# delldu/MaskRCNN

Hardware: AMD Instinct MI355X
Metric: images/sec at 1024x1024, 1000 proposals/img (Mask R-CNN inference hot path) (higher is better)
Workload: dtype f32

## Files before the change

__graft_entry__.py:

```python
import importlib.util
import os
import sys

ROOT = os.path.dirname(os.path.abspath(__file__))
if ROOT not in sys.path:
    sys.path.insert(0, ROOT)


def _load(path, name):
    spec = importlib.util.spec_from_file_location(name, path)
    mod = importlib.util.module_from_spec(spec)
    spec.loader.exec_module(mod)
    return mod


def build() -> None:
    import threading
    from oracle import build_ref, oracle

    def _oracles():
        oracle.build()
        try:
            build_ref.build()
        except Exception as e:
            print(f"[build] oracle/_ref not built: {e}", file=sys.stderr)

    t = threading.Thread(target=_oracles)
    t.start()
    b = _load(os.path.join(ROOT, "maskrcnn_amd", "build.py"), "_mrcnn_build")
    b.build_many([(None, (), ()), ("sync_fuzz", ("-DMRCNN_SYNC_FUZZ", "-DMRCNN_W4_ABLATIONS"), ())])
    _load(os.path.join(ROOT, "maskrcnn", "build_native.py"), "_mrcnn_build_native").build()
    t.join()
    import maskrcnn
    import maskrcnn_amd


def smoke() -> None:
    import torch
    assert torch.cuda.is_available(), "smoke() needs a GPU"
    import maskrcnn
    from maskrcnn_amd import modules, ops
    from maskrcnn_amd.config import InferenceConfig
    from maskrcnn_amd.pipeline import MaskRCNNInference
    from oracle import oracle
    dev = torch.device("cuda:0")
    g = torch.Generator().manual_seed(0)
    c = torch.rand(500, 2, generator=g) * 200
    d = torch.cat([c, c + torch.rand(500, 2, generator=g) * 60 + 2,
                   (torch.randperm(500, generator=g).float() / 500)[:, None]], 1)
    assert torch.equal(maskrcnn.nms(d.to(dev), 0.7).cpu(), oracle.nms(d, 0.7)), "nms mismatch"
    img = torch.randn(1, 32, 24, 24, generator=g)
    bx = torch.rand(16, 4, generator=g)
    bx = torch.cat([torch.minimum(bx[:, :2], bx[:, 2:]), torch.maximum(bx[:, :2], bx[:, 2:])], 1)
    ind = torch.zeros(16, dtype=torch.int32)
    got = maskrcnn.CropFunction(7, 7, 0)(img.to(dev), bx.to(dev), ind.to(dev)).cpu()
    assert torch.equal(got, oracle.crop_forward(img, bx, ind, 0.0, 7, 7)), "crop mismatch"
    cfg = InferenceConfig(image_height=128, image_width=128, backbone="resnet50", pre_nms_limit=100,
                          proposal_count=50, detection_max_instances=10)
    sd = modules.synthetic_state_dict("resnet50")
    net = MaskRCNNInference(sd, cfg, dev)
    x = torch.randn(1, 3, 128, 128, generator=g)
    det, mid = net.predict(x.to(dev), torch.tensor([[0., 0., 128., 128.]], device=dev),
                           return_intermediates=True)
    torch.cuda.synchronize()
    want = oracle.fpn_forward(x, sd, "resnet50")
    worst, rng = 0.0, 0.0
    for w, gt in zip(want, mid["feature_maps"]):
        err = (gt[0].permute(2, 0, 1).cpu() - w[0]).abs().max().item()
        worst, rng = max(worst, err), max(rng, w.abs().max().item())
        assert err <= 1e-4, f"trunk mismatch: max|err| {err:.3e} > 1e-4 abs (max|act| {w.abs().max().item():.2f})"
    print(f"trunk vs oracle: max|err| {worst:.2e} abs at max|act| {rng:.2f}")
    assert det.class_ids.shape == (1, 10) and det.masks.shape == (1, 10, 28, 28, 81)
    print("smoke ok")


if __name__ == "__main__":
    build()
    if "--smoke" in sys.argv:
        smoke()
```

maskrcnn_amd/csrc/conv.hip:

```cpp
#include "conv_common.hpp"

#include <algorithm>
#include <cstdlib>
#include <type_traits>

namespace {

using namespace mrcnn_conv;

struct ConvParams : ConvCommon {
    const float* w;
    const float* w_head;
    int head_n;
};

template <int BM, int BN, int BK>
constexpr size_t conv_lds_bytes() {
    return sizeof(float) * 2 * (BM + BN) * (BK == 16 ? BK : BK + 4);
}

template <int BM, int BN, int WM, int WN, int BK, int MODE, int RES, bool SPLIT = false>
__global__ __launch_bounds__(256, 2) void conv_igemm_f32(const ConvParams p) {
    constexpr bool GENERIC = MODE == 1, PW = MODE == 2;
    constexpr bool SWZ = BK == 16;
    constexpr int LDS_STRIDE = SWZ ? BK : BK + 4;
    constexpr int WTM = BM / WM, WTN = BN / WN;
    constexpr int TM = WTM / 32, TN = WTN / 32;
    constexpr int TPR = BK / 4;
    constexpr int RPP = 256 / TPR;
    constexpr int PA = BM / RPP, PB = BN / RPP;
    static_assert(WM * WN == 4 && TM >= 1 && TN >= 1 && PA >= 1 && PB >= 1, "4 waves");
    extern __shared__ __attribute__((aligned(16))) float smem[];
    float* As = smem;
    float* Bs = smem + 2 * BM * LDS_STRIDE;

    int m0, n0, nt;
    if (!tile_origin(p, BM, BN, m0, n0, nt)) return;
    if (p.row_counts && !tile_has_rows(p, m0, BM)) return;

    const int tid = threadIdx.x, lane = tid & 63, wave = tid >> 6;
    const int wm = wave / WN, wn = wave % WN;
    const int kq = tid % TPR, r0 = tid / TPR;
    constexpr bool EARLY_AFFINE = RES == 0 || RES == 3 || RES == 4;
    AffineRegs<TN> affine;
    if constexpr (EARLY_AFFINE) load_affine<TN, WTN>(p, n0, wn, lane, affine);

    int a_off[PA], a_iy[PA], a_ix[PA];
    row_setup<PA, RPP>(p, m0, r0, a_off, a_iy, a_ix);
    int b_off[PB];
    bool b_ok[PB];
#pragma unroll
    for (int i = 0; i < PB; ++i) {
        const int n = n0 + r0 + RPP * i;
        b_ok[i] = n < p.Cout;
        b_off[i] = (b_ok[i] ? n : 0) * p.K + kq * 4;
    }

    unsigned a_voff[PW ? PA : 1], b_voff[PW ? PB : 1];
    if constexpr (PW) {
#pragma unroll
        for (int i = 0; i < PA; ++i)
            a_voff[i] = (m0 + r0 + RPP * i) < p.M ? static_cast<unsigned>(a_off[i] + kq * 4) * 4u : OOB;
#pragma unroll
        for (int i = 0; i < PB; ++i) b_voff[i] = b_ok[i] ? static_cast<unsigned>(b_off[i]) * 4u : OOB;
    }
    float4 ra[PA], rb[PB];
    const __amdgpu_buffer_rsrc_t x_rsrc = __builtin_amdgcn_make_buffer_rsrc(
        const_cast<float*>(p.x), 0, p.x_bytes, 0x00020000);
    const __amdgpu_buffer_rsrc_t w_rsrc = __builtin_amdgcn_make_buffer_rsrc(
        const_cast<float*>(p.w), 0, p.w_bytes, 0x00020000);
    auto bload = [](const __amdgpu_buffer_rsrc_t& r, unsigned byte_off) -> float4 {
        const u32x4 v = __builtin_amdgcn_raw_buffer_load_b128(r, static_cast<int>(byte_off), 0, 0);
        return make_float4(__uint_as_float(v.x), __uint_as_float(v.y), __uint_as_float(v.z),
                           __uint_as_float(v.w));
    };
    int t_c0 = 0, t_ky = 0, t_kx = 0, t_k0 = 0;
    int cur_tap_off = 0, cur_ky = 0, cur_kx = 0, cur_k0 = 0;
    bool cur_kvalid = true;
    int n_c = 0, n_ky = 0, n_kx = 0;
    int g_ky = 0, g_kx = 0, g_tap_off = 0;
    bool g_kin = true;
    if constexpr (GENERIC) {
        const int tap = (kq * 4) / p.Cin;
        n_c = kq * 4 - tap * p.Cin;
        n_ky = tap / p.KW;
        n_kx = tap - n_ky * p.KW;
    }
    auto begin_load = [&]() {
        cur_k0 = t_k0;
        cur_kvalid = t_k0 < p.K;
        if constexpr (GENERIC) {
            g_ky = n_ky;
            g_kx = n_kx;
            g_tap_off = (n_ky * p.W + n_kx) * p.Cin + n_c;
            g_kin = (t_k0 + kq * 4) < p.K;
            n_c += BK;
            while (n_c >= p.Cin) {
                n_c -= p.Cin;
                if (++n_kx == p.KW) { n_kx = 0; ++n_ky; }
            }
        }
        if constexpr (!GENERIC) {
            cur_ky = t_ky;
            cur_kx = t_kx;
            cur_tap_off = (t_ky * p.W + t_kx) * p.Cin + t_c0 + kq * 4;
            t_c0 += BK;
            if (t_c0 >= p.Cin) {
                t_c0 = 0;
                if (++t_kx == p.KW) { t_kx = 0; ++t_ky; }
            }
        }
        t_k0 += BK;
    };
    auto load_piece = [&](int pc) {
        if constexpr (PW) {
            const int kk = cur_k0 < p.K ? cur_k0 : p.K - BK;
            const bool isa = pc < PA;
            const u32x4 v = __builtin_amdgcn_raw_buffer_load_b128(isa ? x_rsrc : w_rsrc,
                                                                  static_cast<int>(isa ? a_voff[isa ? pc : 0] : b_voff[isa ? 0 : pc - PA]),
                                                                  kk * 4, 0);
            const float4 f = make_float4(__uint_as_float(v.x), __uint_as_float(v.y), __uint_as_float(v.z),
                                         __uint_as_float(v.w));
            if (isa) ra[isa ? pc : 0] = f;
            else rb[isa ? 0 : pc - PA] = f;
            return;
        }
        if (pc < PA) {
            const int i = pc;
            if constexpr (!GENERIC) {
                const bool ok = cur_kvalid &&
                                static_cast<unsigned>(a_iy[i] + cur_ky) < static_cast<unsigned>(p.H) &&
                                static_cast<unsigned>(a_ix[i] + cur_kx) < static_cast<unsigned>(p.W);
                ra[i] = bload(x_rsrc, ok ? static_cast<unsigned>(a_off[i] + cur_tap_off) * 4u : OOB);
            } else {
                const bool ok = g_kin &&
                                static_cast<unsigned>(a_iy[i] + g_ky) < static_cast<unsigned>(p.H) &&
                                static_cast<unsigned>(a_ix[i] + g_kx) < static_cast<unsigned>(p.W);
                ra[i] = bload(x_rsrc, ok ? static_cast<unsigned>(a_off[i] + g_tap_off) * 4u : OOB);
            }
        } else {
            const int i = pc - PA;
            bool ok = b_ok[i] && cur_kvalid;
            if constexpr (GENERIC) ok = ok && (cur_k0 + kq * 4 < p.K);
            rb[i] = bload(w_rsrc, ok ? static_cast<unsigned>(b_off[i] + cur_k0) * 4u : OOB);
        }
    };
    static_assert(!SWZ || RPP % 16 == 0, "swizzle term must not depend on the piece");
    const int kqs = SWZ ? (kq ^ ((r0 >> 2) & 3)) : kq;
    auto store_piece = [&](int pc, int buf) {
        if (pc < PA)
            *reinterpret_cast<float4*>(As + buf * BM * LDS_STRIDE + (r0 + RPP * pc) * LDS_STRIDE + kqs * 4) = ra[pc];
        else
            *reinterpret_cast<float4*>(Bs + buf * BN * LDS_STRIDE + (r0 + RPP * (pc - PA)) * LDS_STRIDE + kqs * 4) =
                rb[pc - PA];
    };
    constexpr int NP = PA + PB;

    f32x16 acc[TM][TN];
#pragma unroll
    for (int i = 0; i < TM; ++i)
#pragma unroll
        for (int j = 0; j < TN; ++j)
#pragma unroll
            for (int r = 0; r < 16; ++r) acc[i][j][r] = 0.f;

    const int nk = (p.K + BK - 1) / BK;
    constexpr int NCH = BK / 8;
    constexpr int NM = 4 * TM * TN;
    static_assert(NCH >= 2, "needs at least two chunks per k tile");
    begin_load();
#pragma unroll
    for (int pc = 0; pc < NP; ++pc) load_piece(pc);
#pragma unroll
    for (int pc = 0; pc < NP; ++pc) store_piece(pc, 0);
    __syncthreads();
    begin_load();
#pragma unroll
    for (int pc = 0; pc < NP; ++pc) load_piece(pc);

    const int fsw = SWZ ? (((lane & 31) >> 2) & 3) : 0;
    const int frow = (lane & 31) * LDS_STRIDE;
    const int fch0 = (((lane >> 5)) ^ fsw) * 4, fch1 = ((2 + (lane >> 5)) ^ fsw) * 4;
    const int frag = frow + (lane >> 5) * 4;
    const float* Aw = As + wm * WTM * LDS_STRIDE + (SWZ ? frow : frag);
    const float* Bw = Bs + wn * WTN * LDS_STRIDE + (SWZ ? frow : frag);
    float4 fa[2][TM], fb[2][TN];
    auto read_frags = [&](int slot, int buf, int j) {
        const int jo = SWZ ? (j == 0 ? fch0 : fch1) : j * 8;
#pragma unroll
        for (int i = 0; i < TM; ++i)
            fa[slot][i] = *reinterpret_cast<const float4*>(Aw + buf * BM * LDS_STRIDE + i * 32 * LDS_STRIDE + jo);
#pragma unroll
        for (int i = 0; i < TN; ++i)
            fb[slot][i] = *reinterpret_cast<const float4*>(Bw + buf * BN * LDS_STRIDE + i * 32 * LDS_STRIDE + jo);
    };
    read_frags(0, 0, 0);
    f32x16 acc2[SPLIT ? TM : 1][SPLIT ? TN : 1];
    if constexpr (SPLIT) {
#pragma unroll
        for (int i = 0; i < TM; ++i)
#pragma unroll
            for (int j = 0; j < TN; ++j)
#pragma unroll
                for (int r = 0; r < 16; ++r) acc2[i][j][r] = 0.f;
    }
    auto ktile = [&](auto chain_tag, int kt) {
        constexpr int CH = decltype(chain_tag)::value;
        const int buf = kt & 1;
#pragma unroll
        for (int j = 0; j < NCH; ++j) {
            const int cur = j & 1;
            if (j + 1 < NCH) {
                read_frags(cur ^ 1, buf, j + 1);
            } else {
                __syncthreads();
                read_frags(cur ^ 1, buf ^ 1, 0);
                begin_load();
            }
            __builtin_amdgcn_sched_barrier(0);
#pragma unroll
            for (int s = 0; s < 4; ++s) {
#pragma unroll
                for (int i = 0; i < TM; ++i) {
                    const float4 a = fa[cur][i];
                    const float av = s == 0 ? a.x : s == 1 ? a.y : s == 2 ? a.z : a.w;
#pragma unroll
                    for (int jn = 0; jn < TN; ++jn) {
                        const float4 b = fb[cur][jn];
                        const float bv = s == 0 ? b.x : s == 1 ? b.y : s == 2 ? b.z : b.w;
                        if constexpr (SPLIT && CH == 1)
                            acc2[i][jn] = __builtin_amdgcn_mfma_f32_32x32x2f32(av, bv, acc2[i][jn], 0, 0, 0);
                        else
                            acc[i][jn] = __builtin_amdgcn_mfma_f32_32x32x2f32(av, bv, acc[i][jn], 0, 0, 0);
                        const int m = (s * TM + i) * TN + jn;
#pragma unroll
                        for (int pc = m * NP / NM; pc < (m + 1) * NP / NM; ++pc) {
                            if (j == NCH - 2) store_piece(pc, buf ^ 1);
                            if (j == NCH - 1) load_piece(pc);
                        }
                        __builtin_amdgcn_sched_barrier(0);
                    }
                }
            }
        }
    };
    if constexpr (!SPLIT) {
        for (int kt = 0; kt < nk; ++kt) ktile(std::integral_constant<int, 0>{}, kt);
    } else {
        constexpr int TPB = 32 / BK;
        static_assert(BK == 32 || BK == 16, "SPLIT: chains are 32-wide k blocks");
        for (int kt = 0; kt < nk; kt += 2 * TPB) {
#pragma unroll
            for (int u = 0; u < TPB; ++u)
                if (kt + u < nk) ktile(std::integral_constant<int, 0>{}, kt + u);
#pragma unroll
            for (int u = 0; u < TPB; ++u)
                if (kt + TPB + u < nk) ktile(std::integral_constant<int, 1>{}, kt + TPB + u);
        }
#pragma unroll
        for (int i = 0; i < TM; ++i)
#pragma unroll
            for (int j = 0; j < TN; ++j)
#pragma unroll
                for (int r = 0; r < 16; ++r) acc[i][j][r] += acc2[i][j][r];
    }

    if constexpr (RES == 5) {
        static_assert(BM == 128 && BN == 128 && WM == 2 && WN == 2, "heads epilogue is written for the 128x128 tile");
        constexpr int TS = BN + 4;
        const int ln = lane & 31, lh = lane >> 5;
        __syncthreads();
        float* T = smem;
#pragma unroll
        for (int jn = 0; jn < TN; ++jn) {
            const int n = n0 + wn * WTN + jn * 32 + ln;
            const float sc = p.scale ? p.scale[n] : 1.0f, sh = p.shift ? p.shift[n] : 0.0f;
#pragma unroll
            for (int i = 0; i < TM; ++i)
#pragma unroll
                for (int r = 0; r < 16; ++r) {
                    float v = acc[i][jn][r] * sc + sh;
                    v = v > 0.f ? v : 0.f;
                    T[(wm * WTM + i * 32 + (r & 3) + 8 * (r >> 2) + 4 * lh) * TS + wn * WTN + jn * 32 + ln] = v;
                }
        }
        __syncthreads();
        f32x16 hacc;
#pragma unroll
        for (int r = 0; r < 16; ++r) hacc[r] = 0.f;
        const float* Trow = T + (wave * 32 + ln) * TS + lh * 4;
        const float* Wrow = p.w_head + static_cast<int64_t>(ln) * p.Cout + n0 + lh * 4;
#pragma unroll 4
        for (int j = 0; j < BN / 8; ++j) {
            const float4 a = *reinterpret_cast<const float4*>(Trow + j * 8);
            const float4 b = *reinterpret_cast<const float4*>(Wrow + j * 8);
            hacc = __builtin_amdgcn_mfma_f32_32x32x2f32(a.x, b.x, hacc, 0, 0, 0);
            hacc = __builtin_amdgcn_mfma_f32_32x32x2f32(a.y, b.y, hacc, 0, 0, 0);
            hacc = __builtin_amdgcn_mfma_f32_32x32x2f32(a.z, b.z, hacc, 0, 0, 0);
            hacc = __builtin_amdgcn_mfma_f32_32x32x2f32(a.w, b.w, hacc, 0, 0, 0);
        }
        const __amdgpu_buffer_rsrc_t o_rsrc = __builtin_amdgcn_make_buffer_rsrc(p.y, 0, p.y_bytes, 0x00020000);
        const unsigned tile_base = static_cast<unsigned>(nt) * static_cast<unsigned>(p.M) * p.head_n * 4u;
#pragma unroll
        for (int r = 0; r < 16; ++r) {
            const int m = m0 + wave * 32 + (r & 3) + 8 * (r >> 2) + 4 * lh;
            const bool ok = m < p.M && ln < p.head_n;
            const unsigned off = ok ? tile_base + (static_cast<unsigned>(m) * p.head_n + ln) * 4u : OOB;
            __builtin_amdgcn_raw_buffer_store_b32(__float_as_uint(hacc[r]), o_rsrc, static_cast<int>(off), 0, 0);
        }
        return;
    }

    ResidualRegs<TM, TN, RES> rv;
    if constexpr (RES == 4) {
        if ((p.Cout & 1) == 0 && ((p.Cout >> 2) & 1) == 0) {
            load_residual_pairs<TM, TN, WTM, WTN, RES>(p, m0, n0, wm, wn, lane, rv);
            epilogue_pairs<TM, TN, WTM, WTN, RES>(p, acc, rv, m0, n0, wm, wn, lane, EARLY_AFFINE ? &affine : nullptr);
            return;
        }
    }
    if constexpr (RES != 5) load_residual<TM, TN, WTM, WTN, RES>(p, m0, n0, wm, wn, lane, rv);
    if constexpr (RES != 5) epilogue<TM, TN, WTM, WTN, RES>(p, acc, rv, m0, n0, wm, wn, lane, EARLY_AFFINE ? &affine : nullptr);
}


template <int KC, int TN, int TNP>
__global__ __launch_bounds__(256, 2) void conv_pw_stream_f32(const ConvParams p) {
    constexpr int K = KC * 8, LDSB = K + 4, NPASS = TN / TNP;
    static_assert(KC % 4 == 0 && TN % TNP == 0, "whole 128-byte lines; whole passes");
    extern __shared__ __attribute__((aligned(16))) float smem[];
    const int tid = threadIdx.x, lane = tid & 63, wave = tid >> 6, ln = lane & 31, lh = lane >> 5;
    const __amdgpu_buffer_rsrc_t x_rsrc = __builtin_amdgcn_make_buffer_rsrc(const_cast<float*>(p.x), 0, p.x_bytes, 0x00020000);
    const __amdgpu_buffer_rsrc_t w_rsrc = __builtin_amdgcn_make_buffer_rsrc(const_cast<float*>(p.w), 0, p.w_bytes, 0x00020000);
    for (int idx = tid; idx < 32 * TN * (K / 4); idx += 256) {
        const int n = idx / (K / 4), c = idx - n * (K / 4);
        const u32x4 v = __builtin_amdgcn_raw_buffer_load_b128(w_rsrc, (n * K + 4 * c) * 4, 0, 0);
        *reinterpret_cast<u32x4*>(smem + n * LDSB + 4 * c) = v;
    }
    AffineRegs<TN> affine;
    load_affine<TN, 32 * TN>(p, 0, 0, lane, affine);
    __syncthreads();

    const int nblocks = (p.M + 31) >> 5;
    const int nw = static_cast<int>(gridDim.x) * 4;
    int blk = static_cast<int>(blockIdx.x) * 4 + wave;
    if (blk >= nblocks) return;
    const unsigned lane_off = static_cast<unsigned>(ln * K + 4 * lh) * 4u;
    auto voff = [&](int b) -> unsigned {
        return (b < nblocks && b * 32 + ln < p.M) ? static_cast<unsigned>(b) * (32u * K * 4u) + lane_off : OOB;
    };
    u32x4 a[KC];
    {
        const unsigned vo = voff(blk);
#pragma unroll
        for (int j = 0; j < KC; ++j)
            a[j] = __builtin_amdgcn_raw_buffer_load_b128(x_rsrc, static_cast<int>(vo == OOB ? OOB : vo + j * 32u), 0, 0);
    }
    const float* Bw = smem + ln * LDSB + lh * 4;
    for (; blk < nblocks; blk += nw) {
        const unsigned vo_next = voff(blk + nw);
#pragma unroll
        for (int ps = 0; ps < NPASS; ++ps) {
            f32x16 acc[1][TNP];
#pragma unroll
            for (int jn = 0; jn < TNP; ++jn)
#pragma unroll
                for (int r = 0; r < 16; ++r) acc[0][jn][r] = 0.f;
            float4 fb[2][TNP];
            auto read_b = [&](int slot, int j) {
#pragma unroll
                for (int jn = 0; jn < TNP; ++jn)
                    fb[slot][jn] = *reinterpret_cast<const float4*>(Bw + (ps * TNP + jn) * 32 * LDSB + j * 8);
            };
            read_b(0, 0);
#pragma unroll
            for (int j = 0; j < KC; ++j) {
                if (j + 1 < KC) read_b((j + 1) & 1, j + 1);
                __builtin_amdgcn_sched_barrier(0);
                const u32x4 av = a[j];
#pragma unroll
                for (int s = 0; s < 4; ++s) {
                    const float af = __uint_as_float(s == 0 ? av.x : s == 1 ? av.y : s == 2 ? av.z : av.w);
#pragma unroll
                    for (int jn = 0; jn < TNP; ++jn) {
                        const float4 b = fb[j & 1][jn];
                        const float bf = s == 0 ? b.x : s == 1 ? b.y : s == 2 ? b.z : b.w;
                        acc[0][jn] = __builtin_amdgcn_mfma_f32_32x32x2f32(af, bf, acc[0][jn], 0, 0, 0);
                        __builtin_amdgcn_sched_barrier(0);
                    }
                }
                if (ps == NPASS - 1 && (j & 3) == 3) {
#pragma unroll
                    for (int jj = j - 3; jj <= j; ++jj)
                        a[jj] = __builtin_amdgcn_raw_buffer_load_b128(
                            x_rsrc, static_cast<int>(vo_next == OOB ? OOB : vo_next + jj * 32u), 0, 0);
                    __builtin_amdgcn_sched_barrier(0);
                }
            }
            AffineRegs<TNP> af;
#pragma unroll
            for (int jn = 0; jn < TNP; ++jn) {
                af.sc[jn] = affine.sc[ps * TNP + jn];
                af.sh[jn] = affine.sh[ps * TNP + jn];
            }
            ResidualRegs<1, TNP, 0> rv;
            epilogue<1, TNP, 32, 32 * TNP, 0>(p, acc, rv, blk * 32, ps * TNP * 32, 0, 0, lane, &af);
        }
    }
}

template <int KC, int TN, int TNP>
int launch_pw_stream(ConvParams p, hipStream_t stream) {
    constexpr size_t lds = sizeof(float) * 32 * TN * (KC * 8 + 4);
    auto kern = conv_pw_stream_f32<KC, TN, TNP>;
    if (int rc = mrcnn::ensure_dynamic_lds(reinterpret_cast<const void*>(kern), lds, "conv_pw_stream")) return rc;
    const int cus = mrcnn::device_cu_count();
    if (cus <= 0) return mrcnn::fail(MRCNN_ERR_LAUNCH, "conv_pw_stream: no device");
    const int nblocks = (p.M + 31) / 32;
    const int grid = std::min(2 * cus, (nblocks + 3) / 4);
    hipLaunchKernelGGL(kern, dim3(static_cast<unsigned>(grid)), dim3(256), lds, stream, p);
    return mrcnn::check_launch("conv_pw_stream_f32");
}

constexpr int SPLIT_MIN_K = 1024;
template <int BM, int BN, int WM, int WN, int BK>
constexpr bool split_tile() {
    return (BM == 128 && BN == 128 && WM == 2 && WN == 2 && BK == 32) || (BM == 128 && BN == 64 && WM == 2 && WN == 2 && BK == 16) ||
           (BM == 128 && BN == 32 && WM == 4 && WN == 1 && BK == 32);
}

template <int BM, int BN, int WM, int WN, int BK>
int launch_conv(ConvParams p, int mode, hipStream_t stream) {
    const bool generic = mode == 1;
    p.tiles_m = (p.M + BM - 1) / BM;
    p.tiles_n = (p.Cout + BN - 1) / BN;
    const long long grid = tile_grid(p);
    if (grid > 0x7fffffffLL) return mrcnn::fail(MRCNN_ERR_UNSUPPORTED, "conv: grid too large");
    constexpr size_t lds = conv_lds_bytes<BM, BN, BK>();
    const int res = epilogue_variant(p, p.w_head != nullptr);
    auto go = [&](auto kern) -> int {
        if (int rc = mrcnn::ensure_dynamic_lds(reinterpret_cast<const void*>(kern), lds, "conv")) return rc;
        hipLaunchKernelGGL(kern, dim3(static_cast<unsigned>(grid)), dim3(256), lds, stream, p);
        return MRCNN_OK;
    };
    int rc;
#ifdef MRCNN_ABLATIONS
    if constexpr (BM == 128 && BN == 128 && WM == 2 && WN == 2 && BK == 32) {
        if (res == 5) {
            if (generic) return mrcnn::fail(MRCNN_ERR_UNSUPPORTED, "conv: fused heads need Cin %% 32 == 0");
            if ((rc = go(conv_igemm_f32<BM, BN, WM, WN, BK, 0, 5>))) return rc;
            return mrcnn::check_launch("conv_igemm_f32<heads>");
        }
    }
#else
    (void)generic;
#endif
    if (res == 5) return mrcnn::fail(MRCNN_ERR_UNSUPPORTED, "conv: the fused-heads epilogue exists in MRCNN_ABLATIONS builds only");
    if constexpr (split_tile<BM, BN, WM, WN, BK>()) {
        static const bool no_split = getenv("MRCNN_CONV_NO_SPLIT") != nullptr;
        if (p.K >= SPLIT_MIN_K && mode != 1 && res <= 2 && !no_split) {
            auto by_res_split = [&](auto mode_tag) -> int {
                constexpr int MD = decltype(mode_tag)::value;
                return res == 0 ? go(conv_igemm_f32<BM, BN, WM, WN, BK, MD, 0, true>)
                     : res == 1 ? go(conv_igemm_f32<BM, BN, WM, WN, BK, MD, 1, true>)
                                : go(conv_igemm_f32<BM, BN, WM, WN, BK, MD, 2, true>);
            };
            rc = mode == 2 ? by_res_split(std::integral_constant<int, 2>{}) : by_res_split(std::integral_constant<int, 0>{});
            if (rc) return rc;
            return mrcnn::check_launch("conv_igemm_f32<split>");
        }
    }
    auto by_res = [&](auto mode_tag) -> int {
        constexpr int MD = decltype(mode_tag)::value;
        return res == 0 ? go(conv_igemm_f32<BM, BN, WM, WN, BK, MD, 0>)
             : res == 1 ? go(conv_igemm_f32<BM, BN, WM, WN, BK, MD, 1>)
             : res == 2 ? go(conv_igemm_f32<BM, BN, WM, WN, BK, MD, 2>)
             : res == 3 ? go(conv_igemm_f32<BM, BN, WM, WN, BK, MD, 3>)
                        : go(conv_igemm_f32<BM, BN, WM, WN, BK, MD, 4>);
    };
    rc = mode == 1 ? by_res(std::integral_constant<int, 1>{})
       : mode == 2 ? by_res(std::integral_constant<int, 2>{})
                   : by_res(std::integral_constant<int, 0>{});
    if (rc) return rc;
    return mrcnn::check_launch("conv_igemm_f32");
}

}

static int run_conv_f32(const float* x, int32_t batch, int32_t height, int32_t width, int32_t cin,
                        const float* w, int32_t cout, int32_t kh, int32_t kw, int32_t stride, int32_t pad_top,
                        int32_t pad_left, int32_t pad_bottom, int32_t pad_right, const float* scale,
                        const float* shift, const float* residual, int32_t res_div, int32_t relu,
                        int32_t out_mode, float* y, mrcnn_stream_t stream, int32_t res_kblocked = 0,
                        const int32_t* row_counts = nullptr, int32_t rows_per_group = 0) {
    MRCNN_REQUIRE(x && w && y, "conv: null pointer");
    ConvParams p;
    if (int rc = fill_common(p, "conv", x, batch, height, width, cin, 4, cout, kh, kw, stride, pad_top, pad_left,
                             pad_bottom, pad_right, scale, shift, residual, res_div, relu, out_mode, y, 4, res_kblocked))
        return rc;
    if (row_counts) {
        MRCNN_REQUIRE(rows_per_group >= 1 && p.M % rows_per_group == 0, "conv: %d output rows are not whole groups of %d",
                      p.M, rows_per_group);
        p.row_counts = row_counts;
        p.rows_per_group = rows_per_group;
    }
    p.w = w;
    p.w_head = nullptr;
    p.head_n = 0;
    const long long M = p.M;
    const bool generic = (cin % 32) != 0;
    static const bool no_pw = mrcnn::tuning_env("MRCNN_CONV_NO_PW") != nullptr;
    const bool pointwise = !generic && kh == 1 && kw == 1 && pad_top == 0 && pad_left == 0 && pad_bottom == 0 &&
                           pad_right == 0 && !no_pw;
    const int mode = generic ? 1 : pointwise ? 2 : 0;
    hipStream_t s = mrcnn::as_stream(stream);
    static const int force = mrcnn::tuning_env("MRCNN_CONV_TILE") ? atoi(mrcnn::tuning_env("MRCNN_CONV_TILE")) : 0;
    static const bool no_stream = mrcnn::tuning_env("MRCNN_CONV_NO_STREAM") != nullptr;
    if (pointwise && !no_stream && !row_counts && stride == 1 && !residual && relu <= 1 && out_mode != 1 && p.M >= 131072) {
        if (cin == 256 && cout > 32 && cout <= 64) return launch_pw_stream<32, 2, 2>(p, s);
        if (cin == 64 && cout > 32 && cout <= 64) return launch_pw_stream<8, 2, 2>(p, s);
        if (cin == 64 && cout > 128 && cout <= 256) return launch_pw_stream<8, 8, 4>(p, s);
    }
    if (cout <= 32) return launch_conv<128, 32, 4, 1, 32>(p, mode, s);
    if (cout <= 64) return (generic || force == 4) ? launch_conv<256, 64, 4, 1, 32>(p, mode, s)
                                                   : launch_conv<256, 64, 4, 1, 16>(p, mode, s);
    if (!generic && force == 0 && cout > 64 && cout <= 96) return launch_conv<128, 96, 4, 1, 32>(p, mode, s);
    if (!generic && (force == 3 || (force == 0 && ((p.K <= 128 && cout >= 256) || (out_mode == 1 && p.K <= 256 && cout >= 256)))))
        return launch_conv<128, 128, 2, 2, 16>(p, mode, s);
    const long long tiles128 = ((p.M + 127) / 128) * static_cast<long long>((cout + 127) / 128);
    const bool underfilled = cout >= 128 && tiles128 < mrcnn::device_cu_count();
    if (!generic && force == 0 && underfilled && p.K >= 1024 &&
        ((p.M + 127) / 128) * static_cast<long long>((cout + 63) / 64) <= mrcnn::device_cu_count())
        return launch_conv<128, 32, 4, 1, 32>(p, mode, s);
    if (!generic && force != 1 &&
        (force == 5 || underfilled || (p.K <= 256 && p.residual && p.res_div == 1 && cout >= 128)))
        return launch_conv<128, 64, 2, 2, 16>(p, mode, s);
    return launch_conv<128, 128, 2, 2, 32>(p, mode, s);
}

extern "C" int mrcnn_conv_bn_act_nhwc_f32(const float* x, int32_t batch, int32_t height, int32_t width,
                                          int32_t cin, const float* w, int32_t cout, int32_t kh,
                                          int32_t kw, int32_t stride, int32_t pad_top, int32_t pad_left,
                                          int32_t pad_bottom, int32_t pad_right, const float* scale,
                                          const float* shift, const float* residual, int32_t res_div,
                                          int32_t activation, float* y, mrcnn_stream_t stream) {
    return run_conv_f32(x, batch, height, width, cin, w, cout, kh, kw, stride, pad_top, pad_left, pad_bottom,
                        pad_right, scale, shift, residual, res_div, activation, 0, y, stream);
}

extern "C" int mrcnn_conv_bn_act_f32(const float* x, int32_t batch, int32_t height, int32_t width, int32_t cin,
                                     const float* w, int32_t cout, int32_t kh, int32_t kw, int32_t stride,
                                     int32_t pad_top, int32_t pad_left, int32_t pad_bottom, int32_t pad_right,
                                     const float* scale, const float* shift, const float* residual, int32_t res_div,
                                     int32_t residual_layout, int32_t activation, float* y, int32_t y_layout,
                                     mrcnn_stream_t stream) {
    MRCNN_REQUIRE(y_layout == MRCNN_LAYOUT_NHWC || y_layout == MRCNN_LAYOUT_KBLOCKED, "conv: bad y_layout");
    MRCNN_REQUIRE(residual_layout == MRCNN_LAYOUT_NHWC || residual_layout == MRCNN_LAYOUT_KBLOCKED,
                  "conv: bad residual_layout");
    return run_conv_f32(x, batch, height, width, cin, w, cout, kh, kw, stride, pad_top, pad_left, pad_bottom,
                        pad_right, scale, shift, residual, res_div, activation,
                        y_layout == MRCNN_LAYOUT_KBLOCKED ? 2 : 0, y, stream,
                        residual_layout == MRCNN_LAYOUT_KBLOCKED ? 1 : 0);
}

extern "C" int mrcnn_conv_bn_act_rows_f32(const float* x, int32_t batch, int32_t height, int32_t width, int32_t cin,
                                          const float* w, int32_t cout, int32_t kh, int32_t kw, int32_t stride,
                                          int32_t pad_top, int32_t pad_left, int32_t pad_bottom, int32_t pad_right,
                                          const float* scale, const float* shift, int32_t activation, float* y,
                                          const int32_t* row_counts, int32_t rows_per_group, mrcnn_stream_t stream) {
    MRCNN_REQUIRE(row_counts == nullptr || rows_per_group >= 1, "conv_rows: rows_per_group=%d", rows_per_group);
    return run_conv_f32(x, batch, height, width, cin, w, cout, kh, kw, stride, pad_top, pad_left, pad_bottom, pad_right, scale,
                        shift, nullptr, 1, activation, 0, y, stream, 0, row_counts, rows_per_group);
}

extern "C" int32_t mrcnn_conv_rows_tile_m(int32_t cout) { return (cout > 32 && cout <= 64) ? 256 : 128; }

extern "C" int mrcnn_deconv2x2_bias_act_nhwc_f32(const float* x, int32_t batch, int32_t height, int32_t width,
                                                 int32_t cin, const float* w, int32_t cout, const float* bias4,
                                                 int32_t activation, float* y, mrcnn_stream_t stream) {
    MRCNN_REQUIRE(cout >= 1, "deconv2x2: cout=%d", cout);
    return run_conv_f32(x, batch, height, width, cin, w, 4 * cout, 1, 1, 1, 0, 0, 0, 0, nullptr, bias4, nullptr, 1,
                        activation, 1, y, stream);
}

#ifdef MRCNN_ABLATIONS
namespace {
__global__ __launch_bounds__(256) void heads_reduce(const float* __restrict__ partial, const float* __restrict__ bias,
                                                    int64_t MC, int head_n, int tiles, float* __restrict__ y) {
    for (int64_t e = blockIdx.x * static_cast<int64_t>(blockDim.x) + threadIdx.x; e < MC;
         e += static_cast<int64_t>(gridDim.x) * blockDim.x) {
        float v = bias ? bias[e % head_n] : 0.f;
        for (int t = 0; t < tiles; ++t) v += partial[t * MC + e];
        y[e] = v;
    }
}
}

extern "C" size_t mrcnn_rpn_level_workspace_bytes(int32_t batch, int32_t height, int32_t width, int32_t cout,
                                                  int32_t head_n) {
    if (batch < 1 || height < 1 || width < 1 || cout < 1 || head_n < 1) return 0;
    return sizeof(float) * static_cast<size_t>((cout + 127) / 128) * batch * height * width * head_n;
}

extern "C" int mrcnn_rpn_level_fused_f32(const float* x, int32_t batch, int32_t height, int32_t width, int32_t cin,
                                         const float* w_shared, int32_t cout, const float* b_shared,
                                         const float* w_head32, const float* b_head, int32_t head_n,
                                         void* workspace, size_t workspace_bytes, float* y, mrcnn_stream_t stream) {
    MRCNN_REQUIRE(x && w_shared && w_head32 && workspace && y, "rpn_level: null pointer");
    MRCNN_REQUIRE(batch >= 1 && height >= 1 && width >= 1 && cin % 32 == 0 && cin >= 32,
                  "rpn_level: bad shape (Cin %% 32 == 0 required)");
    MRCNN_REQUIRE(cout % 128 == 0 && cout >= 128, "rpn_level: Cout=%d must be a multiple of 128", cout);
    MRCNN_REQUIRE(head_n >= 1 && head_n <= 32, "rpn_level: head_n=%d must be in [1,32]", head_n);
    MRCNN_REQUIRE(workspace_bytes >= mrcnn_rpn_level_workspace_bytes(batch, height, width, cout, head_n),
                  "rpn_level: workspace too small");
    const long long M = 1LL * batch * height * width;
    const int tiles_n = cout / 128;
    MRCNN_REQUIRE(4 * M * cin <= MAX_BUFFER_BYTES && 36LL * cin * cout <= MAX_BUFFER_BYTES &&
                      4 * M * head_n * tiles_n <= MAX_BUFFER_BYTES,
                  "rpn_level: tensor too large for 32-bit buffer offsets");
    ConvParams p;
    p.x = x; p.w = w_shared; p.scale = nullptr; p.shift = b_shared; p.residual = nullptr;
    p.y = static_cast<float*>(workspace);
    p.B = batch; p.H = height; p.W = width; p.Cin = cin; p.Cout = cout; p.KH = 3; p.KW = 3;
    p.stride = 1; p.pad_t = 1; p.pad_l = 1; p.OH = height; p.OW = width;
    p.M = static_cast<int>(M);
    p.K = 9 * cin;
    p.res_div = 1; p.act = 1; p.out_mode = 0; p.res_kblocked = 0;
    p.ow_shift = p.ohw_shift = -1;
    p.x_bytes = static_cast<unsigned>(4LL * M * cin);
    p.w_bytes = static_cast<unsigned>(4LL * p.K * cout);
    p.y_bytes = static_cast<unsigned>(4LL * tiles_n * M * head_n);
    p.r_bytes = 0;
    p.w_head = w_head32;
    p.head_n = head_n;
    hipStream_t s = mrcnn::as_stream(stream);
    if (int rc = launch_conv<128, 128, 2, 2, 32>(p, 0, s)) return rc;
    const int64_t MC = M * head_n;
    int64_t blocks = (MC + 255) / 256;
    if (blocks > 256 * 16) blocks = 256 * 16;
    hipLaunchKernelGGL(heads_reduce, dim3(static_cast<unsigned>(blocks)), dim3(256), 0, s,
                       static_cast<const float*>(workspace), b_head, MC, head_n, tiles_n, y);
    return mrcnn::check_launch("heads_reduce");
}
#endif
```

Baseline: 419.6.

## Stage conv epilogue through LDS for coalesced 128-bit residual loads and stores

Adds an alternative conv epilogue that writes each wave's accumulators into a per-wave LDS slice after the main loop. It reads them back as contiguous float4 rows, so residual loads and output stores become 128-bit coalesced buffer accesses instead of scattered per-lane 32-bit accesses. By default it is used for half-size residual epilogues and for full residual epilogues with small K, and an env var can force it on or off. It costs an extra block barrier and LDS round trips, and adds more template instantiations and a tuning build variant.

Result: no change. 421.9 (median of 6 runs) (+0.6%).

```diff
diff --git a/__graft_entry__.py b/__graft_entry__.py
--- a/__graft_entry__.py
+++ b/__graft_entry__.py
@@ -28,7 +28,8 @@
     t = threading.Thread(target=_oracles)
     t.start()
     b = _load(os.path.join(ROOT, "maskrcnn_amd", "build.py"), "_mrcnn_build")
-    b.build_many([(None, (), ()), ("sync_fuzz", ("-DMRCNN_SYNC_FUZZ", "-DMRCNN_W4_ABLATIONS"), ())])
+    b.build_many([(None, (), ()), ("sync_fuzz", ("-DMRCNN_SYNC_FUZZ", "-DMRCNN_W4_ABLATIONS"), ()),
+                  ("conv_epilogue", ("-DMRCNN_TUNING",), ("conv.hip",))])
     _load(os.path.join(ROOT, "maskrcnn", "build_native.py"), "_mrcnn_build_native").build()
     t.join()
     import maskrcnn
diff --git a/maskrcnn_amd/csrc/conv.hip b/maskrcnn_amd/csrc/conv.hip
--- a/maskrcnn_amd/csrc/conv.hip
+++ b/maskrcnn_amd/csrc/conv.hip
@@ -19,7 +19,130 @@
     return sizeof(float) * 2 * (BM + BN) * (BK == 16 ? BK : BK + 4);
 }
 
-template <int BM, int BN, int WM, int WN, int BK, int MODE, int RES, bool SPLIT = false>
+template <int TM, int TN, int WTM, int WTN, int RES>
+__device__ __forceinline__ void epilogue_lds(const ConvCommon& p, f32x16 (&acc)[TM][TN], float* slice, int m0, int n0, int wm,
+                                             int wn, int lane, const AffineRegs<TN>* pre) {
+    static_assert(RES >= 0 && RES <= 2, "plain, residual, half-size residual");
+    constexpr int ROWS = TN == 1 ? 32 : 16;
+    constexpr int NH = 32 / ROWS;
+    constexpr int NR = ROWS / 2;
+    constexpr int CG = 8 * TN;
+    constexpr int NQ = ROWS * CG / 64;
+    constexpr int PITCH = 32 * TN;
+    constexpr bool SAMECOL = 64 % CG == 0;
+    static_assert(ROWS * CG % 64 == 0, "whole wave reads");
+    const int ln = lane & 31, lh = lane >> 5;
+    const __amdgpu_buffer_rsrc_t y_rsrc = __builtin_amdgcn_make_buffer_rsrc(p.y, 0, p.y_bytes, 0x00020000);
+    int srow[NQ], n4[NQ];
+#pragma unroll
+    for (int k = 0; k < NQ; ++k) {
+        const int q = lane + 64 * k;
+        srow[k] = q / CG;
+        n4[k] = n0 + wn * WTN + (q % CG) * 4;
+    }
+    u32x4 rv[(RES ? TM : 1)][(RES ? NH : 1)][(RES ? NQ : 1)];
+    if constexpr (RES == 1 || RES == 2) {
+        const __amdgpu_buffer_rsrc_t r_rsrc = __builtin_amdgcn_make_buffer_rsrc(
+            const_cast<float*>(p.residual), 0, p.r_bytes, 0x00020000);
+        const int rh = p.OH >> 1, rw = p.OW >> 1;
+        const unsigned row_bytes = p.res_kblocked ? 32u : static_cast<unsigned>(p.Cout) * 4u;
+        const unsigned rplane = static_cast<unsigned>(RES == 1 ? p.M : p.M >> 2) * 32u;
+        const unsigned rblock = p.res_kblocked ? rplane : 32u;
+        unsigned rcol[NQ];
+#pragma unroll
+        for (int k = 0; k < NQ; ++k) {
+            const unsigned c = static_cast<unsigned>(n4[k] >> 3) * rblock + static_cast<unsigned>(n4[k] & 7) * 4u;
+            rcol[k] = (SAMECOL && k > 0) ? rcol[0] : n4[k] < p.Cout ? c : OOB;
+        }
+#pragma unroll
+        for (int i = 0; i < TM; ++i)
+#pragma unroll
+            for (int h = 0; h < NH; ++h)
+#pragma unroll
+                for (int k = 0; k < NQ; ++k) {
+                    const int m = m0 + wm * WTM + i * 32 + h * ROWS + srow[k];
+                    const bool ok = m < p.M;
+                    unsigned rrow;
+                    if constexpr (RES == 1) {
+                        rrow = ok ? static_cast<unsigned>(m) * row_bytes : OOB;
+                    } else {
+                        const int mm = ok ? m : 0;
+                        int b, oy, ox;
+                        decode_pixel(p, mm, b, oy, ox);
+                        rrow = ok ? static_cast<unsigned>((b * rh + (oy >> 1)) * rw + (ox >> 1)) * row_bytes : OOB;
+                    }
+                    rv[i][h][k] = __builtin_amdgcn_raw_buffer_load_b128(r_rsrc, static_cast<int>(oob_add(rrow, rcol[k])), 0, 0);
+                }
+    }
+    AffineRegs<TN> af;
+    if (pre) af = *pre;
+    else load_affine<TN, WTN>(p, n0, wn, lane, af);
+    const unsigned yblock = p.out_mode == 2 ? static_cast<unsigned>(p.M) * 32u : 32u;
+    unsigned ycol[NQ];
+#pragma unroll
+    for (int k = 0; k < NQ; ++k) {
+        const unsigned c = static_cast<unsigned>(n4[k] >> 3) * yblock + static_cast<unsigned>(n4[k] & 7) * 4u;
+        ycol[k] = (SAMECOL && k > 0) ? ycol[0] : n4[k] < p.Cout ? c : OOB;
+    }
+    const unsigned row_bytes = p.out_mode == 2 ? 32u : static_cast<unsigned>(p.Cout) * 4u;
+    float* wr = slice + 4 * lh * PITCH + ln;
+    const float4* rd = reinterpret_cast<const float4*>(slice) + lane;
+    auto passes = [&](auto act_tag) {
+    constexpr bool ACT = decltype(act_tag)::value;
+#pragma unroll
+    for (int i = 0; i < TM; ++i)
+#pragma unroll
+        for (int h = 0; h < NH; ++h) {
+#pragma unroll
+            for (int jn = 0; jn < TN; ++jn)
+#pragma unroll
+                for (int rr = 0; rr < NR; ++rr)
+                    wr[((rr & 3) + 8 * (rr >> 2)) * PITCH + jn * 32] = acc[i][jn][h * NR + rr] * af.sc[jn] + af.sh[jn];
+            __builtin_amdgcn_fence(__ATOMIC_RELEASE, "wavefront");
+            __builtin_amdgcn_wave_barrier();
+            __builtin_amdgcn_fence(__ATOMIC_ACQUIRE, "wavefront");
+            float4 t[NQ];
+#pragma unroll
+            for (int k = 0; k < NQ; ++k) t[k] = rd[64 * k];
+            __builtin_amdgcn_fence(__ATOMIC_RELEASE, "wavefront");
+            __builtin_amdgcn_wave_barrier();
+            __builtin_amdgcn_fence(__ATOMIC_ACQUIRE, "wavefront");
+#pragma unroll
+            for (int k = 0; k < NQ; ++k) {
+                float v0 = t[k].x, v1 = t[k].y, v2 = t[k].z, v3 = t[k].w;
+                if constexpr (RES == 1 || RES == 2) {
+                    v0 += __uint_as_float(rv[i][h][k].x);
+                    v1 += __uint_as_float(rv[i][h][k].y);
+                    v2 += __uint_as_float(rv[i][h][k].z);
+                    v3 += __uint_as_float(rv[i][h][k].w);
+                }
+                if constexpr (ACT)
+                    asm("v_max_f32 %0, 0, %0\n\tv_max_f32 %1, 0, %1\n\tv_max_f32 %2, 0, %2\n\tv_max_f32 %3, 0, %3"
+                        : "+v"(v0), "+v"(v1), "+v"(v2), "+v"(v3));
+                const int m = m0 + wm * WTM + i * 32 + h * ROWS + srow[k];
+                const unsigned yrow = m < p.M ? static_cast<unsigned>(m) * row_bytes : OOB;
+                const u32x4 o = {__float_as_uint(v0), __float_as_uint(v1), __float_as_uint(v2), __float_as_uint(v3)};
+                __builtin_amdgcn_raw_buffer_store_b128(o, y_rsrc, static_cast<int>(oob_add(yrow, ycol[k])), 0, 0);
+            }
+        }
+    };
+    if (p.act) passes(std::true_type{});
+    else passes(std::false_type{});
+}
+
+inline bool lds_epilogue_applies(const ConvCommon& p, int res) {
+    return res >= 0 && res <= 2 && (p.Cout & 3) == 0;
+}
+inline bool lds_epilogue_routed(const ConvCommon& p, int res) {
+    if (!lds_epilogue_applies(p, res)) return false;
+    if (const char* e = mrcnn::tuning_env("MRCNN_CONV_EPILOGUE")) {
+        if (e[0] == 'l') return true;
+        if (e[0] == 'p') return false;
+    }
+    return res == 2 || (res == 1 && p.K <= 128);
+}
+
+template <int BM, int BN, int WM, int WN, int BK, int MODE, int RES, bool SPLIT = false, bool LDSEPI = false>
 __global__ __launch_bounds__(256, 2) void conv_igemm_f32(const ConvParams p) {
     constexpr bool GENERIC = MODE == 1, PW = MODE == 2;
     constexpr bool SWZ = BK == 16;
@@ -311,6 +434,14 @@
         return;
     }
 
+    if constexpr (LDSEPI) {
+        constexpr int SLICE = (TN == 1 ? 32 : 16) * 32 * TN;
+        static_assert(4 * SLICE * sizeof(float) <= conv_lds_bytes<BM, BN, BK>(), "the four slices fit the operand tiles");
+        __syncthreads();
+        epilogue_lds<TM, TN, WTM, WTN, RES>(p, acc, smem + wave * SLICE, m0, n0, wm, wn, lane, EARLY_AFFINE ? &affine : nullptr);
+        return;
+    }
+
     ResidualRegs<TM, TN, RES> rv;
     if constexpr (RES == 4) {
         if ((p.Cout & 1) == 0 && ((p.Cout >> 2) & 1) == 0) {
@@ -438,6 +569,7 @@
     if (grid > 0x7fffffffLL) return mrcnn::fail(MRCNN_ERR_UNSUPPORTED, "conv: grid too large");
     constexpr size_t lds = conv_lds_bytes<BM, BN, BK>();
     const int res = epilogue_variant(p, p.w_head != nullptr);
+    const bool lds_epi = lds_epilogue_routed(p, res);
     auto go = [&](auto kern) -> int {
         if (int rc = mrcnn::ensure_dynamic_lds(reinterpret_cast<const void*>(kern), lds, "conv")) return rc;
         hipLaunchKernelGGL(kern, dim3(static_cast<unsigned>(grid)), dim3(256), lds, stream, p);
@@ -461,6 +593,10 @@
         if (p.K >= SPLIT_MIN_K && mode != 1 && res <= 2 && !no_split) {
             auto by_res_split = [&](auto mode_tag) -> int {
                 constexpr int MD = decltype(mode_tag)::value;
+                if (lds_epi)
+                    return res == 0 ? go(conv_igemm_f32<BM, BN, WM, WN, BK, MD, 0, true, true>)
+                         : res == 1 ? go(conv_igemm_f32<BM, BN, WM, WN, BK, MD, 1, true, true>)
+                                    : go(conv_igemm_f32<BM, BN, WM, WN, BK, MD, 2, true, true>);
                 return res == 0 ? go(conv_igemm_f32<BM, BN, WM, WN, BK, MD, 0, true>)
                      : res == 1 ? go(conv_igemm_f32<BM, BN, WM, WN, BK, MD, 1, true>)
                                 : go(conv_igemm_f32<BM, BN, WM, WN, BK, MD, 2, true>);
@@ -472,6 +608,10 @@
     }
     auto by_res = [&](auto mode_tag) -> int {
         constexpr int MD = decltype(mode_tag)::value;
+        if (lds_epi)
+            return res == 0 ? go(conv_igemm_f32<BM, BN, WM, WN, BK, MD, 0, false, true>)
+                 : res == 1 ? go(conv_igemm_f32<BM, BN, WM, WN, BK, MD, 1, false, true>)
+                            : go(conv_igemm_f32<BM, BN, WM, WN, BK, MD, 2, false, true>);
         return res == 0 ? go(conv_igemm_f32<BM, BN, WM, WN, BK, MD, 0>)
              : res == 1 ? go(conv_igemm_f32<BM, BN, WM, WN, BK, MD, 1>)
              : res == 2 ? go(conv_igemm_f32<BM, BN, WM, WN, BK, MD, 2>)
@@ -514,7 +654,7 @@
                            pad_right == 0 && !no_pw;
     const int mode = generic ? 1 : pointwise ? 2 : 0;
     hipStream_t s = mrcnn::as_stream(stream);
-    static const int force = mrcnn::tuning_env("MRCNN_CONV_TILE") ? atoi(mrcnn::tuning_env("MRCNN_CONV_TILE")) : 0;
+    const int force = mrcnn::tuning_env("MRCNN_CONV_TILE") ? atoi(mrcnn::tuning_env("MRCNN_CONV_TILE")) : 0;
     static const bool no_stream = mrcnn::tuning_env("MRCNN_CONV_NO_STREAM") != nullptr;
     if (pointwise && !no_stream && !row_counts && stride == 1 && !residual && relu <= 1 && out_mode != 1 && p.M >= 131072) {
         if (cin == 256 && cout > 32 && cout <= 64) return launch_pw_stream<32, 2, 2>(p, s);
```
